# Rodrigops27/MPC-EKF4FastCharge

Measured on AMD Instinct MI355X. Metric: MPC+EKF control steps/sec (whole batch), Np=5 Nc=2; 1/2/4/8 MI355X, higher is better.
Workload: dtype f64

## Files before the change

mpc-ekf4fastcharge_amd/csrc/mpcekf_host.cpp:

```cpp
#include <hip/hip_runtime.h>

#include <sched.h>

#include <algorithm>
#include <cmath>
#include <condition_variable>
#include <cstdarg>
#include <cstdio>
#include <cstdlib>
#include <cstring>
#include <deque>
#include <mutex>
#include <new>
#include <string>
#include <thread>
#include <vector>

#include "../../include/mpcekf.h"
#include "mpcekf_eig.hpp"
#include "mpcekf_kernels.hpp"
#include "mpcekf_summary.hpp"
#include "mpcekf_thermal.hpp"

using namespace mk;
// ... 114 lines not shown
    hipError_t e = err;
    err = hipSuccess;
    return e;
  }
  ~Copier() {
    {
      std::lock_guard<std::mutex> g(mu);
      stop = true;
    }
    cv.notify_all();
    for (std::thread &t : th) t.join();
  }
};

int copy_threads() {
  if (const char *e = std::getenv("MPCEKF_COPY_THREADS")) return std::max(0, std::min(64, std::atoi(e)));
  cpu_set_t set;
  int n = 8;
  if (sched_getaffinity(0, sizeof set, &set) == 0) n = CPU_COUNT(&set);
  return std::max(1, std::min(16, n));
}

}

struct mpcekf_ctx {
  int device = 0;
  hipStream_t stream = nullptr;
  int64_t n = 0;
  int NM = 0, nz = 0, nzp = 0;
  int ncon = 0, ncon_dev = 0, sw = 7;
  bool initialized = false;
  KRom r{};
  KCfg k{};
  KState s{};
  mpcekf_config cfg{};
  double *d_cell_blob = nullptr, *d_plant_blob = nullptr, *d_bulk = nullptr, *d_poly = nullptr;
  double *d_const = nullptr;
  double *d_mb = nullptr;
  bool mb = false;
  double *d_scal = nullptr;
  int *d_int = nullptr;
  double *d_prob = nullptr;
  double *d_zk = nullptr, *d_zbk = nullptr;
  double *d_bnd = nullptr;
  int *d_xm = nullptr;
  double *d_xg = nullptr;
  bool split_cell = false;
  bool quad = false;
  int ekf4_block = 256;
  int *d_ts = nullptr;
  double *d_hist = nullptr;
  double *d_hot = nullptr;
  int *d_hot_i = nullptr;
  int hot_clear() {
    if (d_hot_i) HIPCHK(hipMemsetAsync(d_hot_i, 0xFF, (size_t)n * 4 * sizeof(int), stream));
    return MPCEKF_OK;
  }
  long long *d_stamps = nullptr;
  bool wide = false;
  KWide w{};
  double *d_lin = nullptr, *d_zsoc = nullptr;
  std::vector<double> h_lim;
  double *d_lim = nullptr;
  bool percell = false;
  const double *lim() const { return percell ? d_lim : nullptr; }
  double *d_sum = nullptr, *d_sum_reach = nullptr, *d_sum_obs = nullptr;
  char *d_sum_ring = nullptr;
  int32_t sum_slot = -1;
  size_t sum_row() const { return (((size_t)SUM_WIN * (size_t)n * 8) + 255) & ~(size_t)255; }
  double *d_th = nullptr, *d_th_par = nullptr, *d_th_i = nullptr, *d_th_ocv = nullptr;
  int32_t th_nocv = 0;
  double *d_uk1p = nullptr;
  int flush_period = LAZY_H;
  bool flush_roll = false;
  hipStream_t fstream = nullptr;
  hipEvent_t ev_fork = nullptr, ev_join = nullptr;
  bool bounds_side = false;
  hipEvent_t ev_bfork = nullptr, ev_bjoin = nullptr;
  double *d_tmp = nullptr;
  size_t tmp_bytes = 0;
  char *h_bounce = nullptr;
  size_t h_bytes = 0, bounce_max = (size_t)256 << 20;
  size_t xoff = 0, xchunk = (size_t)4 << 20, xhwm = 0;
  std::vector<hipEvent_t> xev;
  size_t xev_used = 0;
  bool xpending = false;
  Copier *copier = nullptr;
  hipError_t next_event(hipEvent_t *e) {
    if (xev_used == xev.size()) {
      hipEvent_t ne = nullptr;
      hipError_t r = hipEventCreateWithFlags(&ne, hipEventDisableTiming);
      if (r != hipSuccess) return r;
      xev.push_back(ne);
    }
    *e = xev[xev_used++];
    return hipSuccess;
  }
  int drain() {
    hipError_t e = hipStreamSynchronize(stream);
    hipError_t c = copier ? copier->drain() : hipSuccess;
    xoff = 0;
    xev_used = 0;
    xpending = false;
    if (e != hipSuccess) return fail(MPCEKF_E_HIP, "hipStreamSynchronize: %s", hipGetErrorString(e));
    if (c != hipSuccess) return fail(MPCEKF_E_HIP, "output copy: %s", hipGetErrorString(c));
    return MPCEKF_OK;
  }
  bool timing = false;
// ... 657 lines not shown
  hipError_t e = hipStreamCreateWithFlags(&X->stream, hipStreamNonBlocking);
  if (e == hipSuccess && (X->flush_roll || X->bounds_side)) {
    e = hipStreamCreateWithFlags(&X->fstream, hipStreamNonBlocking);
    if (e == hipSuccess) e = hipEventCreateWithFlags(&X->ev_fork, hipEventDisableTiming);
    if (e == hipSuccess) e = hipEventCreateWithFlags(&X->ev_join, hipEventDisableTiming);
    if (e == hipSuccess) e = hipEventCreateWithFlags(&X->ev_bfork, hipEventDisableTiming);
    if (e == hipSuccess) e = hipEventCreateWithFlags(&X->ev_bjoin, hipEventDisableTiming);
  }
  if (e != hipSuccess) { mpcekf_ctx_destroy(X); return fail(MPCEKF_E_HIP, "stream: %s", hipGetErrorString(e)); }
  const size_t n = (size_t)ncells, NM = (size_t)X->NM;
  KState &s = X->s;
  s.n = ncells;
  if ((rc = dalloc(&s.bigx, n * NM * 6)) || (rc = dalloc(&s.ekf, n * NM * REC)) ||
      (rc = dalloc(&X->d_scal, n * 10)) || (rc = dalloc(&s.lam, n * X->ncon_dev)) ||
      (rc = hipMalloc((void **)&X->d_int, (n * 4 + 1) * sizeof(int)) == hipSuccess ? 0 : MPCEKF_E_HIP) || (rc = dalloc(&X->d_prob, n * PROB_DOUBLES)) || (rc = dalloc(&X->d_const, n * 8)) ||
      (rc = dalloc(&X->d_zk, n * (X->nz + 2))) || (rc = dalloc(&X->d_zbk, n * (X->nz + 2))) ||
      (rc = dalloc(&X->d_bnd, n * NBND)) || (rc = dalloc(&X->d_xg, n * 4)) ||
      (rc = hipMalloc((void **)&X->d_xm, n * 4 * sizeof(int)) == hipSuccess ? 0 : MPCEKF_E_HIP) ||
      (rc = dalloc(&X->d_ts, n * NM * 2)) || (rc = dalloc(&X->d_hist, n * LAZY_H * 2)) ||
      (X->mb && (rc = dalloc(&X->d_mb, n * MBREC)))
#ifdef MPCEKF_STAMPS
      || (rc = dalloc(&X->d_stamps, n * NSTAMPS))
#endif
  ) {
    mpcekf_ctx_destroy(X);
    return rc;
  }
  double *sc = X->d_scal;
  s.SOCn = sc; s.SOCp = sc + n; s.x0 = sc + 2 * n; s.S0 = sc + 3 * n; s.priorI = sc + 4 * n;
  s.uk_1 = sc + 5 * n; s.uk = sc + 6 * n; s.vk = sc + 7 * n; s.J_unc = sc + 8 * n; s.J_fin = sc + 9 * n;
  s.warn = X->d_int; s.status = X->d_int + n; s.nviol = X->d_int + 2 * n; s.hflag = X->d_int + 3 * n;
  s.hslow = X->d_int + 4 * n;
  HIPCHK(hipMemset(s.hslow, 0, sizeof(int)));
  s.prob = X->d_prob;
  s.ts_ekf = X->d_ts; s.ts_plant = X->d_ts + n * NM;
  s.hist_p = X->d_hist; s.hist_u = X->d_hist + n * LAZY_H;
  s.mb = X->d_mb;
  s.stamps = X->d_stamps;
  {
    bool hot = true;
    if (const char *e = std::getenv("MPCEKF_HOT_CORNERS")) hot = std::atoi(e) != 0;
    if (hot && !X->mb && !X->quad && !X->flush_roll && n > 0) {
      if (hipMalloc((void **)&X->d_hot, n * 4 * REC * sizeof(double)) != hipSuccess ||
          hipMalloc((void **)&X->d_hot_i, n * 8 * sizeof(int)) != hipSuccess) {
        (void)hipGetLastError();
        if (X->d_hot) (void)hipFree(X->d_hot);
        if (X->d_hot_i) (void)hipFree(X->d_hot_i);
        X->d_hot = nullptr;
        X->d_hot_i = nullptr;
      } else {
        s.hot_rec = X->d_hot;
        s.hot_m = X->d_hot_i;
        s.hot_ts = X->d_hot_i + n * 4;
        if ((rc = X->hot_clear())) { mpcekf_ctx_destroy(X); return rc; }
      }
    }
  }
  if (X->d_stamps) HIPCHK(hipMemset(X->d_stamps, 0, (size_t)n * NSTAMPS * sizeof(long long)));
  double *cs = X->d_const;
  s.Tc = cs; s.SOC0 = cs + n; s.SOC0n = cs + 2 * n; s.SOC0p = cs + 3 * n;
  if (X->sw != 7 && ((rc = dalloc(&X->d_lin, n * MPCEKF_LIN_SIZE)) || (rc = dalloc(&X->d_zsoc, n)))) {
    mpcekf_ctx_destroy(X);
    return rc;
  }
  if (X->wide) {
    KWide &w = X->w;
    w.Np = cfg->Np; w.Nc = cfg->Nc; w.ncon = X->ncon;
    const size_t nc = (size_t)X->ncon;
    if ((rc = dalloc(&w.prob, n * wide_prob_doubles(w.Np, w.Nc))) || (rc = dalloc(&w.X, nc * n * w.Nc)) ||
        (rc = dalloc(&w.R, (size_t)n * (w.Nc * (w.Nc + 1) / 2))) || (rc = dalloc(&w.K, nc * n)) || (rc = dalloc(&w.hii, nc * n)) || (rc = dalloc(&w.it, n)) ||
        (rc = dalloc(&w.smin, (size_t)w.Nc * w.Nc + 1)) || (rc = dalloc(&X->d_lin, n * MPCEKF_LIN_SIZE)) ||
        (rc = dalloc(&w.q, 1)) || (rc = dalloc(&w.list, n)) || (rc = dalloc(&w.hist, 128)) ||
        (rc = dalloc(&X->d_zsoc, n))) {
      mpcekf_ctx_destroy(X);
      return rc;
    }
    HIPCHK(hipMemset(w.q, 0, sizeof(int)));
    HIPCHK(hipMemset(w.hist, 0, 128 * sizeof(int)));
    HIPCHK(hipMemset(w.it, 0, n * sizeof(int)));
    rc = launch_wide_smin(w, -rom->Ts / (3600 * rom->Q), rom->A, X->stream);
    if (rc) { mpcekf_ctx_destroy(X); return fail(MPCEKF_E_HIP, "smin kernel: %s", hipGetErrorString((hipError_t)rc)); }
    HIPCHK(hipStreamSynchronize(X->stream));
  }
  *out = X;
  return MPCEKF_OK;
}

int mpcekf_ctx_destroy(mpcekf_ctx *X) {
  if (!X) return MPCEKF_OK;
  (void)hipSetDevice(X->device);
  if (X->stream) (void)X->drain();
  if (X->fstream) (void)hipStreamSynchronize(X->fstream);
  delete X->copier;
  X->copier = nullptr;
  for (hipEvent_t e : X->xev) (void)hipEventDestroy(e);
  for (hipEvent_t e : X->ev) (void)hipEventDestroy(e);
  if (X->ev_fork) (void)hipEventDestroy(X->ev_fork);
  if (X->ev_join) (void)hipEventDestroy(X->ev_join);
  if (X->ev_bfork) (void)hipEventDestroy(X->ev_bfork);
  if (X->ev_bjoin) (void)hipEventDestroy(X->ev_bjoin);
  void *ptrs[] = {X->d_prob, X->d_cell_blob, X->d_plant_blob, X->d_bulk, X->d_const, X->d_scal, X->d_int, X->d_zk,
                  X->d_zbk,       X->d_tmp,        X->s.bigx, X->s.ekf,   X->s.lam,   X->d_ts, X->d_hist, X->d_stamps, X->d_bnd, X->d_xm, X->d_xg,
                  X->w.prob, X->w.X, X->w.R, X->w.K, X->w.hii, X->w.it, X->w.smin, X->d_lin, X->d_zsoc, X->d_mb, X->d_uk1p,
                  X->w.q, X->w.list, X->w.hist, X->d_poly, X->d_szk, X->d_sxg, X->d_sxm, X->d_slin, X->d_sv, X->d_zslot,
                  X->d_obs_blob, X->d_obs, X->d_obs_plan, X->d_lim, X->d_sum, X->d_sum_reach, X->d_sum_obs,
                  X->d_sum_ring, X->d_th, X->d_th_par, X->d_th_i, X->d_th_ocv, X->d_hot, X->d_hot_i};
  for (void *p : ptrs)
    if (p) (void)hipFree(p);
  for (auto &g : X->graphs) (void)hipGraphExecDestroy(g.exec);
  if (X->h_bounce) (void)hipHostFree(X->h_bounce);
  if (X->fstream) (void)hipStreamDestroy(X->fstream);
  if (X->stream) (void)hipStreamDestroy(X->stream);
  delete X;
  return MPCEKF_OK;
}

int mpcekf_ctx_config(const mpcekf_ctx *X, mpcekf_config *cfg) {
  if (!X || !cfg) return fail(MPCEKF_E_ARG, "ctx_config: null argument");
  *cfg = X->cfg;
  return MPCEKF_OK;
}

int mpcekf_ctx_info(const mpcekf_ctx *X, int64_t *ncells, int32_t *nmodels, int32_t *nz, int32_t *ncon) {
  if (!X) return fail(MPCEKF_E_ARG, "null ctx");
  if (ncells) *ncells = X->n;
  if (nmodels) *nmodels = X->NM;
  if (nz) *nz = X->nz;
  if (ncon) *ncon = X->ncon;
  return MPCEKF_OK;
}

static double host_soc(const mpcekf_ctx *X, int side, double z, double T) {
  const std::vector<double> &tk = X->tabT;
  const int nte = (int)tk.size();
  const std::vector<double> &a = X->soc_end[side][0], &b = X->soc_end[side][1];
  if (nte == 1) return a[0] + z * (b[0] - a[0]);
  const double Tc = std::fmin(std::fmax(T, tk[0]), tk[nte - 1]);
  int j = 0;
  while (j < nte - 2 && Tc >= tk[j + 1]) ++j;
  const double g = (Tc - tk[j]) / (tk[j + 1] - tk[j]);
  const double s0 = a[j] + g * (a[j + 1] - a[j]), s1 = b[j] + g * (b[j + 1] - b[j]);
  return s0 + z * (s1 - s0);
}

static int check_tc(const double *tc, size_t count) {
  for (size_t i = 0; i < count; ++i)
    if (!(tc[i] <= 100) || !std::isfinite(tc[i]))
      return fail(MPCEKF_E_ARG, "temperature %zu = %g: must be finite and in degC (iterEKF.m:62)", i, tc[i]);
  return MPCEKF_OK;
}

static int set_tc(mpcekf_ctx *X, const double *tc, struct Xfer *xf = nullptr);

int mpcekf_init_cells(mpcekf_ctx *X, const double *soc0_pct, const double *tc_degC) {
  if (X) X->stage_zk = X->stage_lin = X->stage_v = X->stage_obs = false;
  if (!X || ((!soc0_pct || !tc_degC) && X->n)) return fail(MPCEKF_E_ARG, "init_cells: null argument");
  HIPCHK(hipSetDevice(X->device));
  const size_t n = (size_t)X->n;
  int rc0 = 0;
// ... 288 lines not shown
      if (slice && fork) HIPCHK(hipStreamWaitEvent(X->stream, X->ev_join, 0));
      if (roll ? t == nsteps : (t % P == 0 || t == nsteps)) {
        const bool timed = E && !roll;
        if (timed) HIPCHK(hipEventRecord(E[5], X->stream));
        if ((rc = lerr(launch_flush(X->r, X->k, X->s, t, t == nsteps ? 0 : t, X->stream), "flush"))) return rc;
        if (timed) HIPCHK(hipEventRecord(E[6], X->stream));
        flushed[k] = timed;
      }
      if (sum && ((size_t)t % ring == 0 || t == nsteps)) {
        KSum q{};
        q.rec = X->d_sum;
        q.reach = X->d_sum_reach;
        q.u = (const double *)f[0].dev;
        q.v = (const double *)f[1].dev;
        q.soc = (const double *)f[2].dev;
        q.phise = (const double *)f[3].dev;
        q.nexec = (const int *)f[4].dev;
        q.obs = (const double *)f[14].dev;
        q.n = X->n;
        q.nrows = (int)((size_t)k % ring) + 1;
        q.max_hild = X->cfg.max_hild;
        if ((rc = lerr(launch_summary(q, X->stream), "summary"))) return rc;
      }
      if (thermal) {
        KTherm q{};
        q.Tc = X->s.Tc;
        q.vk = X->s.vk;
        q.SOCn = X->s.SOCn;
        q.status = X->s.status;
        q.uk = X->s.uk;
        q.iapp = X->d_th_i;
        q.par = X->d_th_par;
        q.ocv = X->d_th_ocv;
        q.rec = X->d_th;
        q.temp = (double *)row(15, k);
        q.heat = (double *)row(16, k);
        q.n = X->n;
        q.nocv = X->th_nocv;
        q.th0n = X->r.th0n;
        q.th100n = X->r.th100n;
        q.Ts = X->r.Ts;
        if ((rc = lerr(launch_thermal(q, X->stream), "thermal"))) return rc;
      }
    }
    return MPCEKF_OK;
  };
  if (capturing) {
    std::vector<uintptr_t> key = {(uintptr_t)nsteps, (uintptr_t)dtc, (uintptr_t)diag, (uintptr_t)bounds};
    for (const F &e : f) key.push_back((uintptr_t)e.dev);
    key.push_back((uintptr_t)osel.plan);
    key.push_back((uintptr_t)nslots);
    key.push_back((uintptr_t)lim);
    key.push_back((uintptr_t)X->s.hot_rec);
    for (int i = 0; i < nslots; ++i) key.push_back((uintptr_t)slots[i]);
    key.push_back((uintptr_t)X->d_th_ocv);
    key.push_back((uintptr_t)X->th_nocv);
    key.push_back((uintptr_t)X->d_th);
    key.push_back((uintptr_t)(sum ? X->d_sum_reach : nullptr));
    key.push_back((uintptr_t)(sum ? X->d_sum : nullptr));
    if ((rc = X->graph_launch(key, run_steps))) return rc;
  } else if ((rc = run_steps())) {
    return rc;
  }
  if (!outputs_on_device)
    for (int i = 0; i < NF; ++i)
      if (f[i].host)
        HIPCHK(hipMemcpyAsync(f[i].host, f[i].dev, per * f[i].width * f[i].esz, hipMemcpyDeviceToHost, X->stream));
  if (nsteps > 0 && f[6].dev)
    HIPCHK(hipMemcpyAsync(X->d_zk, row(6, nsteps - 1), n * nzz * 8, hipMemcpyDeviceToDevice, X->stream));
  if (nsteps > 0 && f[7].dev)
    HIPCHK(hipMemcpyAsync(X->d_zbk, row(7, nsteps - 1), n * nzz * 8, hipMemcpyDeviceToDevice, X->stream));
  HIPCHK(hipStreamSynchronize(X->stream));
  if (X->timing) {
    static const int slot[5] = {MPCEKF_K_PLANT, MPCEKF_K_CELL, MPCEKF_K_BOUNDS, MPCEKF_K_HILD, MPCEKF_K_FLUSH};
    static const int e0[5] = {0, 1, 2, 3, 5};
    for (int k = 0; k < nsteps; ++k)
      for (int j = 0; j < 5; ++j) {
        if ((k + 1) % X->timing_every != 0 && k != nsteps - 1) continue;
        if ((j == 4 && !flushed[k]) || (j == 2 && !bnd_kernel) || (j == 0 && plant_in_cell && !nslots)) continue;
        float ms = 0;
        const int a = j == 3 ? hstart : e0[j], b = j == 3 ? 4 : e0[j] + 1;
        HIPCHK(hipEventElapsedTime(&ms, X->ev[(size_t)k * NEV + a], X->ev[(size_t)k * NEV + b]));
        X->t_ms[slot[j]] += ms;
        X->t_n[slot[j]] += 1;
      }
  }
  return MPCEKF_OK;
}

int mpcekf_step_ex(mpcekf_ctx *X, int32_t nsteps, const double *tc_degC, const mpcekf_traj *tr,
                   int32_t outputs_on_device) {
  return step_impl(X, nsteps, tc_degC, tr, nullptr, 0, nullptr, outputs_on_device);
}

int mpcekf_step_ex_obs(mpcekf_ctx *X, int32_t nsteps, const double *tc_degC, const mpcekf_traj *tr,
                       const int32_t *slots, int32_t nslots, double *obs, int32_t outputs_on_device) {
  return step_impl(X, nsteps, tc_degC, tr, slots, nslots, obs, outputs_on_device);
}

int mpcekf_cl_eig(int32_t n, const double *a, double *re, double *im, double *sv) {
  if (n < 1 || n > mk::eig::MAXN || !a) return fail(MPCEKF_E_ARG, "cl_eig: n must be 1..%d", mk::eig::MAXN);
  double r[mk::eig::MAXN], m[mk::eig::MAXN], s[mk::eig::MAXN];
  if (re || im) mk::eig::eigvals(n, a, r, m);
  if (sv) mk::eig::singvals(n, a, s);
  for (int i = 0; i < n; ++i) {
    if (re) re[i] = r[i];
// ... 1011 lines not shown
```

mpc-ekf4fastcharge_amd/csrc/mpcekf_kernels.hip:

```cpp
#include <hip/hip_runtime.h>

#include <cmath>
#include <cstdlib>
#include <cstdint>
#include <type_traits>

#include "mpcekf_kernels.hpp"
#include "mpcekf_mpc.hpp"
#include "mpcekf_hild.hpp"

#pragma clang fp contract(off)

namespace mk {


#ifdef MPCEKF_STAMPS
#define STAMP(i)                                                                          \
  do {                                                                                    \
    if (io.stamps) io.stamps[(size_t)(i) * s.n + c] = (long long)__builtin_amdgcn_s_memtime(); \
  } while (0)
#define STAMPP(i)                                                                                  \
  do {                                                                                             \
    if (s.stamps) s.stamps[(size_t)(12 + (i)) * s.n + c] = (long long)__builtin_amdgcn_s_memtime(); \
  } while (0)
// ... 941 lines not shown
  }
  if (n2 > 0) {
    double2 v[B];
#pragma unroll
    for (int b = 0; b < B; ++b) v[b] = s2[min(i + b * nt, n2 - 1)];
#pragma unroll
    for (int b = 0; b < B; ++b) d2[min(i + b * nt, n2 - 1)] = v[b];
  }
  if ((len & 1) && threadIdx.x == 0) dst[len - 1] = src[len - 1];
}

#ifndef MPCEKF_RING_CHUNK
#define MPCEKF_RING_CHUNK 8
#endif
constexpr int RCH = MPCEKF_RING_CHUNK;
__device__ __forceinline__ void ring_chunk(const double *ring, const KState &s, int64_t c, int k0, int kmax,
                                           double v[RCH]) {
#pragma unroll
  for (int i = 0; i < RCH; ++i) v[i] = ring[(size_t)(min(k0 + i, kmax) % LAZY_H) * s.n + c];
}
struct PlantCorners {
  int iZu, iZl, iTu, iTl;
};
__device__ __forceinline__ PlantCorners plant_corners(const KRom &r, const double *Tp, const double *Zp,
                                                      double cellSOC, double T) {
  int iZu = 0, iZl = 0, iTu = 0, iTl = 0;
  if (r.nZ > 1) {
    int a, b;
    two_nearest(Zp, r.nZ, cellSOC, a, b);
    iZu = a > b ? a : b; iZl = a < b ? a : b;
  }
  if (r.nT > 1) {
    int a, b;
    two_nearest(Tp, r.nT, T, a, b);
    iTu = a > b ? a : b; iTl = a < b ? a : b;
  }
  return {iZu, iZl, iTu, iTl};
}
__device__ __forceinline__ int corner_model(const KRom &r, const PlantCorners &pc, int j) {
  return ((j & 2) ? pc.iTu : pc.iTl) * r.nZ + ((j & 1) ? pc.iZu : pc.iZl);
}
__device__ __forceinline__ void corner_models(const KRom &r, const PlantCorners &pc, int mm[4]) {
#pragma unroll
  for (int j = 0; j < 4; ++j) mm[j] = corner_model(r, pc, j);
}
__device__ __forceinline__ void plant_weights(const double *Tp, const double *Zp, const PlantCorners &pc,
                                              double cellSOC, double T, double &aZ, double &aT) {
  const double Zu = Zp[pc.iZu], Zl = Zp[pc.iZl], Tu = Tp[pc.iTu], Tl = Tp[pc.iTl];
  aZ = 0.0;
  aT = 0.0;
  if (Zu != Zl) aZ = (cellSOC - Zl) / (Zu - Zl);
  if (Tu != Tl) aT = (T - Tl) / (Tu - Tl);
}
__device__ __forceinline__ void load_corner(const double *bx, double xs[6]) {
  const double2 *p = reinterpret_cast<const double2 *>(bx);
  const double2 q0 = p[0], q1 = p[1], q2 = p[2];
  xs[0] = q0.x; xs[1] = q0.y; xs[2] = q1.x; xs[3] = q1.y; xs[4] = q2.x; xs[5] = q2.y;
}
__device__ __forceinline__ void store_corner(double *bx, const double x[6]) {
  double2 *p = reinterpret_cast<double2 *>(bx);
  p[0] = make_double2(x[0], x[1]);
  p[1] = make_double2(x[2], x[3]);
  p[2] = make_double2(x[4], x[5]);
}
__device__ __forceinline__ void plant_soc_step(const KRom &r, const ETab &et, double SOC0n, double SOC0p, double Iapp,
                                               double &SOCnAvg, double &SOCpAvg) {
  const double Cdleffn = et.f(0, EF_CDL, SOC0n), Cdleffp = et.f(1, EF_CDL, SOC0p);
  double dUn = et.f(0, EF_DU, SOCnAvg), dUp = et.f(1, EF_DU, SOCpAvg);
  double dQn = fabs(r.th100n - r.th0n), dQp = fabs(r.th100p - r.th0p);
  double res0n = -dQn / (3600 * r.Q - Cdleffn * dQn * dUn);
  double res0p = dQp / (3600 * r.Q - Cdleffp * dQp * dUp);
  SOCnAvg = SOCnAvg + res0n * Iapp * r.Ts;
  SOCpAvg = SOCpAvg + res0p * Iapp * r.Ts;
  if (SOCnAvg < 0) SOCnAvg = 0;
  if (SOCnAvg > 1) SOCnAvg = 1;
  if (SOCpAvg < 0) SOCpAvg = 0;
  if (SOCpAvg > 1) SOCpAvg = 1;
}
template <bool A5>
__device__ __forceinline__ void plant_advance(const double *a, const double xs[6], double u, double x[6]) {
#pragma unroll
  for (int e = 0; e < NX; ++e) x[e] = __builtin_fma(a[e], xs[e], u);
  x[NX] = __builtin_fma(A5 ? a[NX] : 1.0, xs[NX], u);
}
template <bool A5>
__device__ __forceinline__ void plant_replay(double xs[6], const double *a, const KState &s, int64_t c, int tsj,
                                             int lazy_t) {
  for (int k0 = tsj + 1; k0 < lazy_t; k0 += RCH) {
    double u[RCH];
    ring_chunk(s.hist_u, s, c, k0, lazy_t - 1, u);
#pragma unroll
    for (int i = 0; i < RCH; ++i)
      if (k0 + i < lazy_t) plant_advance<A5>(a, xs, u[i], xs);
  }
}
__device__ __forceinline__ double plant_row(const double *C, double r0, double d, const double xs[6], double Iapp) {
  double acc = 0.0;
#pragma unroll
  for (int k = 0; k < NX; ++k) acc = acc + C[k] * xs[k];
  acc = acc + r0 * xs[5];
  return acc + d * Iapp;
}
__device__ __forceinline__ double obs_row(const double *B, const double xs[6], double Iapp) {
  const double2 *p = reinterpret_cast<const double2 *>(B);
  const double2 c01 = p[0], c23 = p[1], c4r = p[2], d = p[3];
  double acc = 0.0;
  acc = acc + c01.x * xs[0];
  acc = acc + c01.y * xs[1];
  acc = acc + c23.x * xs[2];
  acc = acc + c23.y * xs[3];
  acc = acc + c4r.x * xs[4];
  acc = acc + c4r.y * xs[5];
  return acc + d.x * Iapp;
}
__device__ __forceinline__ double blend4(double y0, double y1, double y2, double y3, double aZ, double aT) {
  return (1 - aT) * ((1 - aZ) * y0 + aZ * y1) + aT * ((1 - aZ) * y2 + aZ * y3);
// ... 76 lines not shown
  STAMPP(3);
  const double *B = L + mj * PREC;
  double yk[NPLANT];
#pragma unroll
  for (int q = 0; q < NPLANT; ++q) {
    yk[q] = quad_blend(plant_row(B + q * NX, B[NPLANT * NX + q], B[NPLANT * NX + NPLANT + q], xs, Iapp), aZ, aT);
    __builtin_amdgcn_sched_barrier(0);
  }
  STAMPP(4);
  const double V = plant_vcell(r, et, yk, T, Iapp, negSOC, posSOC, SOC0n, SOC0p);
  STAMPP(5);
  if (j == 0) {
    s.SOCn[c] = SOCnAvg;
    s.SOCp[c] = SOCpAvg;
    vout[c] = V;
  }
  if (lazy_t && tsj < lazy_t) {
    double x[6];
    plant_advance<true>(a, xs, Iapp, x);
    store_corner(bx, x);
    s.ts_plant[c * r.NM + mj] = lazy_t;
  }
  STAMPP(6);
}

struct ObsBlob {
  const double *tb, *L, *Tp, *Zp;
};
template <bool GR>
__device__ __forceinline__ ObsBlob obs_stage(const KObs &o, double *lds) {
  const int lo = GR ? o.tab : 0;
  stage_lds(lds, o.blob + lo, o.len - lo);
  __syncthreads();
  const double *tb = lds - lo;
  const double *Tp = tb + o.tab + o.tablen;
  return {tb, GR ? o.blob : lds, Tp, Tp + MAXT};
}
struct ObsCell {
  double negSOC, posSOC, SOC0n, SOC0p, cellSOC, aZ, aT;
  ETab et;
  double xs[6];
  const double *B;
  int mj;
};
template <bool PL>
__device__ __forceinline__ void obs_cell(const KRom &r, const KState &s, const KObs &o, const ObsBlob &ob, int64_t c,
                                         int j, double T, ObsCell &k, int *tsj = nullptr) {
  k.negSOC = s.SOCn[c], k.posSOC = s.SOCp[c];
  k.SOC0n = s.SOC0n[c], k.SOC0p = s.SOC0p[c];
  k.et = etab<PL>(r, ob.tb + o.tab, T);
  k.cellSOC = (k.negSOC - r.th0n) / (r.th100n - r.th0n);
  const PlantCorners pc = plant_corners(r, ob.Tp, ob.Zp, k.cellSOC, T);
  k.mj = corner_model(r, pc, j);
  load_corner(s.bigx + ((size_t)c * r.NM + k.mj) * 6, k.xs);
  if (tsj) *tsj = s.ts_plant[c * r.NM + k.mj];
  plant_weights(ob.Tp, ob.Zp, pc, k.cellSOC, T, k.aZ, k.aT);
  k.B = ob.L + (size_t)k.mj * o.stride;
}
__device__ __forceinline__ double obs_correct(int kind, double v, const ObsCell &k, double UocpnAvg, double UocppAvg,
                                              double negPhise0, double V) {
  switch (kind) {
    case OBS_NTHSS: return fmin(fmax(v + k.SOC0n, 1e-6), 1 - 1e-6);
    case OBS_PTHSS: return fmin(fmax(v + k.SOC0p, 1e-6), 1 - 1e-6);
    case OBS_NPHISE: return v + UocpnAvg;
    case OBS_PPHISE: return v + UocppAvg;
    case OBS_PHIE: return v - negPhise0;
    case OBS_THETAE: return fmax(v + 1, 1e-6);
    case OBS_PPHIS: return v + V;
    default: return v;
  }
}
constexpr int OBS_BLOCK = 512;
template <bool GR, bool PL>
__global__ void __launch_bounds__(OBS_BLOCK) k_plant_obs(const KRom r, const KState s, const KObs o,
                                                            const double *iapp) {
  extern __shared__ double lds[];
  const int64_t gt = (int64_t)blockIdx.x * blockDim.x + threadIdx.x;
  const int j = (int)(gt & 3);
  const int64_t c = gt >> 2;
  const ObsBlob ob = obs_stage<GR>(o, lds);
  if (c >= s.n) return;
  const size_t n = (size_t)s.n;
  double *rec = o.rec + c;
  auto put = [&](int slot, double v) {
    if ((slot & 3) == j) rec[(size_t)slot * n] = v;
  };
  if (s.status[c] & ST_ERROR) {
    for (int k = j; k < o.nobs; k += 4) rec[(size_t)k * n] = __builtin_nan("");
    return;
  }
  const double Iapp = iapp[c];
  const double T = s.Tc[c] + 273.15;
  ObsCell k;
  obs_cell<PL>(r, s, o, ob, c, j, T, k);
  double yk[R_PHISE0 + 1];
#pragma unroll
  for (int q = 0; q <= R_PHISE0; ++q) {
    yk[q] = quad_blend(obs_row(k.B + q * OBS_ROW, k.xs, Iapp), k.aZ, k.aT);
    __builtin_amdgcn_sched_barrier(0);
  }
  const double V = plant_vcell(r, k.et, yk, T, Iapp, k.negSOC, k.posSOC, k.SOC0n, k.SOC0p);
  __builtin_amdgcn_sched_barrier(0);
  const double UocpnAvg = k.et.f(0, EF_U, k.negSOC), UocppAvg = k.et.f(1, EF_U, k.posSOC);
  const double negPhise0 = yk[R_PHISE0] + UocpnAvg;
  __builtin_amdgcn_sched_barrier(0);
  put(OBS_S_NEGSOC, k.negSOC);
  put(OBS_S_POSSOC, k.posSOC);
  put(OBS_S_CELLSOC, k.cellSOC);
// ... 85 lines not shown
  for (int64_t c = blockIdx.x; c < s.n; c += gridDim.x) {
    if (do_ekf) {
      double pri = s.priorI[c];
      double2 *base = reinterpret_cast<double2 *>(s.ekf + (size_t)c * ne);
      for (int j = threadIdx.x; j < ne / 2; j += blockDim.x) {
        int e0 = (2 * j) % REC;
        double2 v = base[j];
        double add0 = e0 < NX ? pri : W;
        double add1 = e0 + 1 < NX ? pri : W;
        v.x = __builtin_fma(cC[2 * j], v.x, add0);
        v.y = __builtin_fma(cC[2 * j + 1], v.y, add1);
        base[j] = v;
      }
    }
    if (do_plant) {
      double u = iapp[c];
      double2 *base = reinterpret_cast<double2 *>(s.bigx + (size_t)c * np);
      for (int j = threadIdx.x; j < np / 2; j += blockDim.x) {
        double2 v = base[j];
        v.x = __builtin_fma(cP[2 * j], v.x, u);
        v.y = __builtin_fma(cP[2 * j + 1], v.y, u);
        base[j] = v;
      }
    }
  }
}

__device__ __forceinline__ double rl64(double v, int l) {
  const long long b = __double_as_longlong(v);
  const int lo = __builtin_amdgcn_readlane((int)b, l), hi = __builtin_amdgcn_readlane((int)(b >> 32), l);
  return __longlong_as_double(((long long)hi << 32) | (long long)(unsigned)lo);
}
__global__ void __launch_bounds__(256) k_flush(const KRom r, const KCfg cf, const KState s, const int t,
                                               const int new_ts, const int64_t c_lo, const int64_t c_hi) {
  const int NM = r.NM;
  const int lane = threadIdx.x & 63;
  const int64_t nw = (int64_t)gridDim.x * (blockDim.x >> 6);
  const int64_t w0 = ((int64_t)blockIdx.x * blockDim.x + threadIdx.x) >> 6;
  const double W = cf.SigmaW;
  const double *cC = r.bulk_tab, *cP = r.bulk_tab + (size_t)NM * REC;
  for (int m0 = 0; m0 < NM; m0 += 64) {
    const int m = m0 + lane;
    const bool act = m < NM;
    const int mm = act ? m : NM - 1;
    double ce[REC], cp[6];
#pragma unroll
    for (int e = 0; e < REC; ++e) ce[e] = cC[(size_t)mm * REC + e];
#pragma unroll
    for (int e = 0; e < 6; ++e) cp[e] = cP[(size_t)mm * 6 + e];
    struct FCell {
      double hpl, hul, xe[REC], xp[6];
      int tse, tsp;
      int slot;
    };
    auto fload = [&](int64_t c, FCell &F) {
      F.hpl = s.hist_p[(size_t)(lane & (LAZY_H - 1)) * s.n + c];
      F.hul = s.hist_u[(size_t)(lane & (LAZY_H - 1)) * s.n + c];
      F.slot = -1;
      if (s.hot_m) {
#pragma unroll
        for (int j = 0; j < 4; ++j)
          if (act && s.hot_m[(size_t)j * s.n + c] == m) F.slot = j;
      }
      const int *tp = F.slot >= 0 ? s.hot_ts + (size_t)F.slot * s.n + c : s.ts_ekf + c * NM + mm;
      F.tse = (act && !(cf.flags & KF_MB)) ? *tp : t;
      F.tsp = act ? s.ts_plant[c * NM + m] : t;
      const double2 *re = reinterpret_cast<const double2 *>(F.slot >= 0 ? hot_slot(s, F.slot, c)
                                                                        : s.ekf + ((size_t)c * NM + mm) * REC);
      const size_t rst = F.slot >= 0 ? (size_t)s.n : 1;
      const double2 *rp = reinterpret_cast<const double2 *>(s.bigx + ((size_t)c * NM + mm) * 6);
#pragma unroll
      for (int e = 0; e < REC / 2; ++e) {
        const double2 v = re[e * rst];
        F.xe[2 * e] = v.x;
        F.xe[2 * e + 1] = v.y;
      }
#pragma unroll
      for (int e = 0; e < 3; ++e) {
        const double2 v = rp[e];
        F.xp[2 * e] = v.x;
        F.xp[2 * e + 1] = v.y;
      }
    };
    FCell cur;
    if (c_lo + w0 < c_hi) fload(c_lo + w0, cur);
    for (int64_t c = c_lo + w0; c < c_hi; c += nw) {
      FCell nx;
      if (c + nw < c_hi) fload(c + nw, nx);
      const double hpl = cur.hpl, hul = cur.hul;
      const int tse = cur.tse, tsp = cur.tsp;
      double2 *re = reinterpret_cast<double2 *>(s.ekf + ((size_t)c * NM + mm) * REC);
      double2 *rp = reinterpret_cast<double2 *>(s.bigx + ((size_t)c * NM + mm) * 6);
      double *xe = cur.xe, *xp = cur.xp;
      int kmin = min(tse, tsp);
#pragma unroll
      for (int o = 1; o < 64; o <<= 1) kmin = min(kmin, __shfl_xor(kmin, o));
      for (int k = kmin + 1; k <= t; ++k) {
        const int sl = k & (LAZY_H - 1);
        const double p = rl64(hpl, sl), u = rl64(hul, sl);
        if (k > tse) {
#pragma unroll
          for (int e = 0; e < NX; ++e) xe[e] = __builtin_fma(ce[e], xe[e], p);
#pragma unroll
          for (int e = NX; e < REC; ++e) xe[e] = __builtin_fma(ce[e], xe[e], W);
        }
        if (k > tsp) {
#pragma unroll
          for (int e = 0; e < 6; ++e) xp[e] = __builtin_fma(cp[e], xp[e], u);
        }
      }
      if (tse < t || cur.slot >= 0) {
#pragma unroll
        for (int e = 0; e < REC / 2; ++e) re[e] = make_double2(xe[2 * e], xe[2 * e + 1]);
      }
      if (cur.slot >= 0) s.hot_m[(size_t)cur.slot * s.n + c] = -1;
      if (tsp < t) {
#pragma unroll
        for (int e = 0; e < 3; ++e) rp[e] = make_double2(xp[2 * e], xp[2 * e + 1]);
      }
      if (act) {
        s.ts_ekf[c * NM + m] = new_ts;
        s.ts_plant[c * NM + m] = new_ts;
      }
      cur = nx;
    }
  }
}

__device__ __forceinline__ void replay_x(double x[NX], const double *a, int ts, int t, double pt, const KState &s,
                                        int64_t c) {
  if (ts + 1 < t) {
    for (int k0 = ts + 1; k0 < t; k0 += RCH) {
      double p[RCH];
      ring_chunk(s.hist_p, s, c, k0, t - 1, p);
#pragma unroll
      for (int i = 0; i < RCH; ++i)
        if (k0 + i < t)
#pragma unroll
          for (int e = 0; e < NX; ++e) x[e] = __builtin_fma(a[e], x[e], p[i]);
    }
  }
  if (ts < t)
#pragma unroll
    for (int e = 0; e < NX; ++e) x[e] = __builtin_fma(a[e], x[e], pt);
}
__device__ __forceinline__ void replay_S(double S[NPK], const double *a, int ts, int t, double W) {
  for (int k = ts + 1; k <= t; ++k) {
#pragma unroll
    for (int i = 0, pp = 0; pp < NX; ++pp)
#pragma unroll
      for (int q = pp; q < NX; ++q, ++i) S[i] = __builtin_fma(a[NX + i], S[i], W);
  }
}

template <int NZ>
__device__ __forceinline__ void ekf_catch_up4(const KState &s, const CellCtx &cc, int NM, const int m[4], int64_t c,
                                              int t, double W, double pt, const bool held[4]) {
  int ts[4];
#pragma unroll
  for (int j = 0; j < 4; ++j) ts[j] = held[j] ? t : s.ts_ekf[c * NM + m[j]];
  bool need[4];
#pragma unroll
  for (int j = 0; j < 4; ++j) {
    need[j] = ts[j] < t;
#pragma unroll
    for (int i = 0; i < j; ++i) need[j] = need[j] && m[i] != m[j];
  }
  if (!(need[0] || need[1] || need[2] || need[3])) return;
  double x[4][NX], S[4][NPK];
// ... 163 lines not shown
    return;
  }
  double V[NA6 * NA6], w[NA6];
  jacobi6(a, V);
#pragma unroll
  for (int k = 0; k < NA6; ++k) w[k] = fabs(a[pk6(k, k)]);
#pragma unroll
  for (int rr = 0; rr < NA6; ++rr)
#pragma unroll
    for (int cI = rr; cI < NA6; ++cI) {
      double hrc = 0.0, hcr = 0.0;
#pragma unroll
      for (int k = 0; k < NA6; ++k) {
        hrc = hrc + (V[rr * NA6 + k] * w[k]) * V[cI * NA6 + k];
        hcr = hcr + (V[cI * NA6 + k] * w[k]) * V[rr * NA6 + k];
      }
      double v = (((P[rr * NA6 + cI] + P[cI * NA6 + rr]) + hrc) + hcr) / 4.0;
      if (bump) v = v * 2.0;
      S[rr * NA6 + cI] = v;
      S[cI * NA6 + rr] = v;
    }
}

__device__ __forceinline__ double qform(const double T[NPK], const double rw[NX]) {
  double q = 0.0;
#pragma unroll
  for (int k = 0; k < NX; ++k) {
    double u = T[pk(k, k)] * rw[k];
#pragma unroll
    for (int l = k + 1; l < NX; ++l) u = __builtin_fma(T[pk(k, l)], rw[l], u);
    q = k == 0 ? rw[0] * u : __builtin_fma(rw[k], u, q);
  }
  return q;
}

template <int NZ, bool PL>
__device__ __forceinline__ double cell_plant(const KRom &r, const KState &s, const double *L, const double *tb,
                                             const double *Tp, const double *Zp, int64_t c, int lazy_t, double Iapp,
                                             double tcs, int st, double &ring_p) {
  constexpr int OA = NZ * NX + NZ, OR0 = NZ * NX + NZ + NX + NPK, OD = NZ * NX;
  const int stride = r.cell_stride;
  if (lazy_t) ring_p = s.priorI[c];
  if (st & ST_ERROR) return __builtin_nan("");
  const double T = tcs + 273.15;
  const ETab et = etab<PL>(r, tb + r.cell_tab, T);
  double SOCnAvg = s.SOCn[c], SOCpAvg = s.SOCp[c];
  const double SOC0n = s.SOC0n[c], SOC0p = s.SOC0p[c];
  const double negSOC = SOCnAvg, posSOC = SOCpAvg;
  double cellSOC = (SOCnAvg - r.th0n) / (r.th100n - r.th0n);
  const PlantCorners pc = plant_corners(r, Tp, Zp, cellSOC, T);
  int mm[4];
  corner_models(r, pc, mm);
  double *bx = s.bigx + (size_t)c * r.NM * 6;
  double xs[4][6];
  int tsj[4] = {0, 0, 0, 0};
#pragma unroll
  for (int j = 0; j < 4; ++j) {
    load_corner(bx + (size_t)mm[j] * 6, xs[j]);
    if (lazy_t) tsj[j] = s.ts_plant[c * r.NM + mm[j]];
  }
  plant_soc_step(r, et, SOC0n, SOC0p, Iapp, SOCnAvg, SOCpAvg);
  if (lazy_t) {
#pragma unroll
    for (int j = 0; j < 4; ++j) plant_replay<false>(xs[j], L + mm[j] * stride + OA, s, c, tsj[j], lazy_t);
  }
  double y[4][NPLANT];
#pragma unroll
  for (int j = 0; j < 4; ++j) {
    const double *B = L + mm[j] * stride;
#pragma unroll
    for (int q = 0; q < NPLANT; ++q) {
      y[j][q] = plant_row(B + q * NX, B[OR0 + q], B[OD + q], xs[j], Iapp);
      launder(y[j][q]);
    }
    __builtin_amdgcn_sched_barrier(0);
  }
  double aZ, aT;
  plant_weights(Tp, Zp, pc, cellSOC, T, aZ, aT);
  double yk[NPLANT];
#pragma unroll
  for (int q = 0; q < NPLANT; ++q) yk[q] = blend4(y[0][q], y[1][q], y[2][q], y[3][q], aZ, aT);
  const double V = plant_vcell(r, et, yk, T, Iapp, negSOC, posSOC, SOC0n, SOC0p);
  s.SOCn[c] = SOCnAvg;
  s.SOCp[c] = SOCpAvg;
  if (lazy_t) {
#pragma unroll
    for (int j = 0; j < 4; ++j) {
      if (tsj[j] >= lazy_t) continue;
      double x[6];
      plant_advance<false>(L + mm[j] * stride + OA, xs[j], Iapp, x);
      store_corner(bx + (size_t)mm[j] * 6, x);
      s.ts_plant[c * r.NM + mm[j]] = lazy_t;
    }
  }
  return V;
}

template <int NZ, int PARTS, bool MB = false, bool GR = false, bool PL = false>
__global__ void __launch_bounds__(256) k_cell(const KRom r, const KCfg cf, const KState s, const KIO io) {
  extern __shared__ double lds[];
  const int lo = GR ? r.cell_tab : 0;
  stage_lds(lds, r.cell_blob + lo, r.cell_len - lo);
  __syncthreads();
  const double *tb = lds - lo;
  const double *Tp = tb + r.cell_tab + r.cell_tablen;
  const double *Zp = Tp + MAXT;
  const int64_t c = (int64_t)blockIdx.x * blockDim.x + threadIdx.x;
  double ring_u = 0.0, ring_p = 0.0;
  bool ring_late = false;
  auto body = [&]() {
  if (c >= s.n) return;
  const int nz = r.nz;
  const double NaN = __builtin_nan("");
  CellCtx cc;
  cc.L = GR ? r.cell_blob : lds;
  cc.Tp = Tp;
  cc.Zp = Zp;
  cc.erec = s.ekf + (size_t)c * r.NM * REC;
  cc.stride = r.cell_stride;
  const bool fplant = (PARTS & P_EKF) && !MB && io.plant;
  const double Tc = fplant && io.tc_in ? io.tc_in[c] : s.Tc[c];
  if (fplant && io.tc_in) s.Tc[c] = Tc;
  cc.T = Tc > 100 ? Tc : Tc + 273.15;
  cc.et = etab<PL>(r, tb + r.cell_tab, cc.T);
  int st = s.status[c];
  const bool fused = io.mode & MODE_FUSED;
  if (io.mode & (MODE_MPC | MODE_FUSED)) s.hflag[c] = 0;
  STAMP(0);

  auto fail_outputs = [&]() {
    if (io.u) io.u[c] = NaN;
    if (io.v) io.v[c] = NaN;
    if (io.soc) io.soc[c] = NaN;
    if (io.phise) io.phise[c] = NaN;
    if (io.nexec) io.nexec[c] = 0;
    if (io.zk)
      for (int q = 0; q < nz + 2; ++q) io.zk[c * (nz + 2) + q] = NaN;
    if (io.zbk)
      for (int q = 0; q < nz + 2; ++q) io.zbk[c * (nz + 2) + q] = NaN;
    if (io.bnd) io.bnd[BD_M * s.n + c] = -1.0;
    if (io.uk_out) io.uk_out[c] = NaN;
    if (io.x_out)
      for (int q = 0; q < 6; ++q) io.x_out[c * 6 + q] = NaN;
    if (io.junc_out) io.junc_out[c] = NaN;
    if (io.jfin_out) io.jfin_out[c] = NaN;
// ... 1529 lines not shown
```

mpc-ekf4fastcharge_amd/csrc/mpcekf_kernels.hpp:

```cpp
#pragma once
#include <cstddef>
#include <cstdint>

namespace mk {

constexpr int NX = 5;
constexpr int NPK = 15;
constexpr int NA = 7;
constexpr int REC = 20;
constexpr int MAXT = 8;
constexpr int MAXZ = 40;
constexpr int MAXROWS = 64;
constexpr int NPLANT = 9;
constexpr int PREC = NPLANT * NX + NPLANT + NPLANT + 6;
#ifndef MPCEKF_LAZY_H
#define MPCEKF_LAZY_H 64
#endif
constexpr int LAZY_H = MPCEKF_LAZY_H;
constexpr int MAXTT = 8;
constexpr int MBREC = 42;
constexpr int KF_MB = 1 << 8;

enum { R_IFDL0 = 0, R_IFDL3, R_IF0, R_IF3, R_TH0, R_TH3, R_TE1, R_TEE, R_PHIE, R_PHISE0, R_NPHISE2, NROLE };
enum : unsigned { G_NTH = 1, G_PTH = 2, G_NPHISE = 4, G_PPHISE = 8, G_PHIE = 16, G_PHIE0 = 32, G_THETAE = 64,
// ... 1 lines not shown
enum { C0_ZERO = 0, C0_CHATV0, C0_RES0N, C0_RES0P, C0_DUN, C0_DUP, C0_MDUN };
enum { ST_ERROR = 1, ST_LOCKOUT = 2, ST_THETAE_NEG = 4 };

struct KRom {
  int NM, nT, nZ, nz, nzp;
  int nth, nte;
  double Ts, Q, F, R, Rc, Tref;
  double th0n, th100n, th0p, th100p;
  unsigned char flags[MAXROWS];
  unsigned fmask[8];
  unsigned char c0k[MAXROWS];
  short perm[MAXROWS];
  const double *cell_blob;
  int cell_stride, cell_tab, cell_tablen, cell_len;
  const double *plant_blob;
  int plant_tab, plant_tablen, plant_len;
  const double *bulk_tab;
  int rom_global;
  int cell_plant;
  int npoly, arr, nodes;
  const double *poly;
};
constexpr int KPOLY = 6;
constexpr int KDESC = 4;
constexpr int KMAP = 4;

struct KCfg {
  double SigmaV, SigmaW, ref, u_max, u_min, du_min, du_max, v_max, phise_min, zmax, hild_tol;
  int max_warn, max_hild, flags;
};

enum { LK_REF = 0, LK_U_MAX, LK_U_MIN, LK_DU_MIN, LK_DU_MAX, LK_V_MAX, LK_PHISE_MIN, LK_ZMAX, NLIMK };

struct KState {
  int64_t n;
  double *bigx;
  double *ekf;
  double *SOCn, *SOCp, *x0, *S0, *priorI, *uk_1, *uk, *vk;
  double *lam;
  int *warn, *status;
  double *Tc;
  const double *SOC0, *SOC0n, *SOC0p;
  double *J_unc, *J_fin;
  int *nviol;
  int *hflag;
  int *hslow;
  double *prob;
  double *mb;
  int *ts_ekf, *ts_plant;
  double *hist_p, *hist_u;
  long long *stamps;
  double *hot_rec;
  int *hot_m, *hot_ts;
};
constexpr int HOT_PAIRS = REC / 2;

constexpr int OBS_ROW = 8;
constexpr int OBS_MAXROWS = 32;
enum { OBS_PLAIN = 0, OBS_NTHSS, OBS_PTHSS, OBS_NPHISE, OBS_PPHISE, OBS_PHIE, OBS_THETAE, OBS_PPHIS };
enum { OBS_S_NEGSOC = 0, OBS_S_POSSOC, OBS_S_CELLSOC };
struct KObs {
  const double *blob;
  int stride, tab, tablen, len;
  int global;
  int nobs, slot_phie0;
  unsigned desc[OBS_MAXROWS];
  double *rec;
};

enum { OBS_SRC_NEGSOC = -1, OBS_SRC_POSSOC = -2, OBS_SRC_CELLSOC = -3, OBS_SRC_PHIE0 = -4, OBS_SRC_VCELL = -5 };
enum { OBS_NEED_V = 1,
       OBS_NEED_UN = 2,
       OBS_NEED_UP = 4 };
struct KObsSel {
  const int *plan;
  int nsel, need;
  double *out;
};

struct KIO {
  int mode;
  double *u, *v, *soc, *phise;
  int *nexec;
  double *zk, *zbk;
  const double *vk_in, *ik_in;
  int *xm_out; double *xg_out;
  const double *zk_in; const int *xm_in; const double *xg_in;
  double *lin_out; const double *lin_in;
  const double *soc_k1_in; double *uk_out;
  int lazy_t;
  double *bnd;
  long long *stamps;
  double *zsoc_out;
  double *x_out;
  double *junc_out, *jfin_out, *normdu_out;
  int *nviol_out;
  int plant;
  const double *tc_in;
};
constexpr int NSTAMPS = 20;
enum { BD_G = 0, BD_M = 4, BD_K = 8, BD_C0 = 14, BD_R0N, BD_R0P, BD_DUN, BD_DUP, BD_S0, NBND };

enum { MODE_EKF = 1, MODE_LIN = 2, MODE_MPC = 4, MODE_FUSED = 8 };
enum { P_EKF = 1, P_MPC = 2, P_ALL = 3, P_LIN = 4 };

struct KWide {
  int Np, Nc, ncon;
  double *prob;
// ... 68 lines not shown
```

Baseline: 269.2 million.

## Add hot-corner cache for plant state in SoA layout

Adds a per-cell four-slot cache for the plant model's active corner states, stored structure-of-arrays (strided by n) so accesses coalesce across cells, mirroring the existing EKF hot-corner cache. On a tag hit the plant step reads and writes the cached slots, and on a miss it spills them back to the bigx array. The flush kernel now checks both EKF and plant tags through lane broadcasts and prefetches the next cell's tags. This adds tag checks, spill logic and extra memory, and risks divergence when cells frequently change corners.

```diff
diff --git a/mpc-ekf4fastcharge_amd/csrc/mpcekf_host.cpp b/mpc-ekf4fastcharge_amd/csrc/mpcekf_host.cpp
--- a/mpc-ekf4fastcharge_amd/csrc/mpcekf_host.cpp
+++ b/mpc-ekf4fastcharge_amd/csrc/mpcekf_host.cpp
@@ -190,8 +190,11 @@
   double *d_hist = nullptr;
   double *d_hot = nullptr;
   int *d_hot_i = nullptr;
+  double *d_hotp = nullptr;
+  int *d_hotp_i = nullptr;
   int hot_clear() {
     if (d_hot_i) HIPCHK(hipMemsetAsync(d_hot_i, 0xFF, (size_t)n * 4 * sizeof(int), stream));
+    if (d_hotp_i) HIPCHK(hipMemsetAsync(d_hotp_i, 0xFF, (size_t)n * 4 * sizeof(int), stream));
     return MPCEKF_OK;
   }
   long long *d_stamps = nullptr;
@@ -955,9 +958,25 @@
         s.hot_rec = X->d_hot;
         s.hot_m = X->d_hot_i;
         s.hot_ts = X->d_hot_i + n * 4;
-        if ((rc = X->hot_clear())) { mpcekf_ctx_destroy(X); return rc; }
       }
     }
+    bool hotp = true;
+    if (const char *e = std::getenv("MPCEKF_HOT_PLANT")) hotp = std::atoi(e) != 0;
+    if (hotp && !X->mb && !X->quad && !X->flush_roll && X->r.cell_plant && n > 0) {
+      if (hipMalloc((void **)&X->d_hotp, n * 4 * 6 * sizeof(double)) != hipSuccess ||
+          hipMalloc((void **)&X->d_hotp_i, n * 8 * sizeof(int)) != hipSuccess) {
+        (void)hipGetLastError();
+        if (X->d_hotp) (void)hipFree(X->d_hotp);
+        if (X->d_hotp_i) (void)hipFree(X->d_hotp_i);
+        X->d_hotp = nullptr;
+        X->d_hotp_i = nullptr;
+      } else {
+        s.hotp_x = X->d_hotp;
+        s.hotp_m = X->d_hotp_i;
+        s.hotp_ts = X->d_hotp_i + n * 4;
+      }
+    }
+    if ((rc = X->hot_clear())) { mpcekf_ctx_destroy(X); return rc; }
   }
   if (X->d_stamps) HIPCHK(hipMemset(X->d_stamps, 0, (size_t)n * NSTAMPS * sizeof(long long)));
   double *cs = X->d_const;
@@ -1007,7 +1026,7 @@
                   X->w.prob, X->w.X, X->w.R, X->w.K, X->w.hii, X->w.it, X->w.smin, X->d_lin, X->d_zsoc, X->d_mb, X->d_uk1p,
                   X->w.q, X->w.list, X->w.hist, X->d_poly, X->d_szk, X->d_sxg, X->d_sxm, X->d_slin, X->d_sv, X->d_zslot,
                   X->d_obs_blob, X->d_obs, X->d_obs_plan, X->d_lim, X->d_sum, X->d_sum_reach, X->d_sum_obs,
-                  X->d_sum_ring, X->d_th, X->d_th_par, X->d_th_i, X->d_th_ocv, X->d_hot, X->d_hot_i};
+                  X->d_sum_ring, X->d_th, X->d_th_par, X->d_th_i, X->d_th_ocv, X->d_hot, X->d_hot_i, X->d_hotp, X->d_hotp_i};
   for (void *p : ptrs)
     if (p) (void)hipFree(p);
   for (auto &g : X->graphs) (void)hipGraphExecDestroy(g.exec);
@@ -1402,6 +1421,7 @@
     key.push_back((uintptr_t)nslots);
     key.push_back((uintptr_t)lim);
     key.push_back((uintptr_t)X->s.hot_rec);
+    key.push_back((uintptr_t)X->s.hotp_x);
     for (int i = 0; i < nslots; ++i) key.push_back((uintptr_t)slots[i]);
     key.push_back((uintptr_t)X->d_th_ocv);
     key.push_back((uintptr_t)X->th_nocv);
diff --git a/mpc-ekf4fastcharge_amd/csrc/mpcekf_kernels.hip b/mpc-ekf4fastcharge_amd/csrc/mpcekf_kernels.hip
--- a/mpc-ekf4fastcharge_amd/csrc/mpcekf_kernels.hip
+++ b/mpc-ekf4fastcharge_amd/csrc/mpcekf_kernels.hip
@@ -1017,16 +1017,26 @@
   if (Zu != Zl) aZ = (cellSOC - Zl) / (Zu - Zl);
   if (Tu != Tl) aT = (T - Tl) / (Tu - Tl);
 }
-__device__ __forceinline__ void load_corner(const double *bx, double xs[6]) {
+__device__ __forceinline__ void load_corner(const double *bx, double xs[6], size_t st = 1) {
   const double2 *p = reinterpret_cast<const double2 *>(bx);
-  const double2 q0 = p[0], q1 = p[1], q2 = p[2];
+  const double2 q0 = p[0], q1 = p[st], q2 = p[2 * st];
   xs[0] = q0.x; xs[1] = q0.y; xs[2] = q1.x; xs[3] = q1.y; xs[4] = q2.x; xs[5] = q2.y;
 }
-__device__ __forceinline__ void store_corner(double *bx, const double x[6]) {
+__device__ __forceinline__ void store_corner(double *bx, const double x[6], size_t st = 1) {
   double2 *p = reinterpret_cast<double2 *>(bx);
   p[0] = make_double2(x[0], x[1]);
-  p[1] = make_double2(x[2], x[3]);
-  p[2] = make_double2(x[4], x[5]);
+  p[st] = make_double2(x[2], x[3]);
+  p[2 * st] = make_double2(x[4], x[5]);
+}
+__device__ __forceinline__ double *hotp_slot(const KState &s, int j, int64_t c) {
+  return s.hotp_x + 2 * ((size_t)j * HOTP_PAIRS * (size_t)s.n + (size_t)c);
+}
+__device__ __forceinline__ int hotp_find(const KState &s, int64_t c, int m) {
+  int slot = -1;
+#pragma unroll
+  for (int i = 0; i < 4; ++i)
+    if (s.hotp_m[(size_t)i * s.n + c] == m) slot = i;
+  return slot;
 }
 __device__ __forceinline__ void plant_soc_step(const KRom &r, const ETab &et, double SOC0n, double SOC0p, double Iapp,
                                                double &SOCnAvg, double &SOCpAvg) {
@@ -1209,8 +1219,10 @@
   k.cellSOC = (k.negSOC - r.th0n) / (r.th100n - r.th0n);
   const PlantCorners pc = plant_corners(r, ob.Tp, ob.Zp, k.cellSOC, T);
   k.mj = corner_model(r, pc, j);
-  load_corner(s.bigx + ((size_t)c * r.NM + k.mj) * 6, k.xs);
-  if (tsj) *tsj = s.ts_plant[c * r.NM + k.mj];
+  const int slot = tsj && s.hotp_m ? hotp_find(s, c, k.mj) : -1;
+  load_corner(slot >= 0 ? hotp_slot(s, slot, c) : s.bigx + ((size_t)c * r.NM + k.mj) * 6, k.xs,
+              slot >= 0 ? (size_t)s.n : 1);
+  if (tsj) *tsj = *(slot >= 0 ? s.hotp_ts + (size_t)slot * s.n + c : s.ts_plant + c * r.NM + k.mj);
   plant_weights(ob.Tp, ob.Zp, pc, k.cellSOC, T, k.aZ, k.aT);
   k.B = ob.L + (size_t)k.mj * o.stride;
 }
@@ -1402,41 +1414,55 @@
       double hpl, hul, xe[REC], xp[6];
       int tse, tsp;
       int slot;
+      int pslot;
     };
-    auto fload = [&](int64_t c, FCell &F) {
+    const int *tags = lane < 4 ? s.hot_m : s.hotp_m;
+    auto ftag = [&](int64_t c) -> int { return lane < 8 && tags ? tags[(size_t)(lane & 3) * s.n + c] : -1; };
+    auto fload = [&](int64_t c, FCell &F, const int tag) {
       F.hpl = s.hist_p[(size_t)(lane & (LAZY_H - 1)) * s.n + c];
       F.hul = s.hist_u[(size_t)(lane & (LAZY_H - 1)) * s.n + c];
       F.slot = -1;
-      if (s.hot_m) {
-#pragma unroll
-        for (int j = 0; j < 4; ++j)
-          if (act && s.hot_m[(size_t)j * s.n + c] == m) F.slot = j;
+      F.pslot = -1;
+#pragma unroll
+      for (int j = 0; j < 4; ++j) {
+        if (act && __builtin_amdgcn_readlane(tag, j) == m) F.slot = j;
+        if (act && __builtin_amdgcn_readlane(tag, 4 + j) == m) F.pslot = j;
       }
       const int *tp = F.slot >= 0 ? s.hot_ts + (size_t)F.slot * s.n + c : s.ts_ekf + c * NM + mm;
+      const int *tq = F.pslot >= 0 ? s.hotp_ts + (size_t)F.pslot * s.n + c : s.ts_plant + c * NM + mm;
       F.tse = (act && !(cf.flags & KF_MB)) ? *tp : t;
-      F.tsp = act ? s.ts_plant[c * NM + m] : t;
+      F.tsp = act ? *tq : t;
       const double2 *re = reinterpret_cast<const double2 *>(F.slot >= 0 ? hot_slot(s, F.slot, c)
                                                                         : s.ekf + ((size_t)c * NM + mm) * REC);
-      const size_t rst = F.slot >= 0 ? (size_t)s.n : 1;
-      const double2 *rp = reinterpret_cast<const double2 *>(s.bigx + ((size_t)c * NM + mm) * 6);
-#pragma unroll
-      for (int e = 0; e < REC / 2; ++e) {
-        const double2 v = re[e * rst];
+      const double2 *rp = reinterpret_cast<const double2 *>(F.pslot >= 0 ? hotp_slot(s, F.pslot, c)
+                                                                         : s.bigx + ((size_t)c * NM + mm) * 6);
+      const size_t rst = F.slot >= 0 ? (size_t)s.n : 1, pst = F.pslot >= 0 ? (size_t)s.n : 1;
+#pragma unroll
+      for (int e = 0; e < REC / 2; ++e, re += rst) {
+        const double2 v = *re;
         F.xe[2 * e] = v.x;
         F.xe[2 * e + 1] = v.y;
       }
 #pragma unroll
-      for (int e = 0; e < 3; ++e) {
-        const double2 v = rp[e];
+      for (int e = 0; e < 3; ++e, rp += pst) {
+        const double2 v = *rp;
         F.xp[2 * e] = v.x;
         F.xp[2 * e + 1] = v.y;
       }
     };
     FCell cur;
-    if (c_lo + w0 < c_hi) fload(c_lo + w0, cur);
+    int tagn = -1;
+    if (c_lo + w0 < c_hi) {
+      fload(c_lo + w0, cur, ftag(c_lo + w0));
+      if (c_lo + w0 + nw < c_hi) tagn = ftag(c_lo + w0 + nw);
+    }
     for (int64_t c = c_lo + w0; c < c_hi; c += nw) {
       FCell nx;
-      if (c + nw < c_hi) fload(c + nw, nx);
+      if (c + nw < c_hi) {
+        const int tag = tagn;
+        if (c + 2 * nw < c_hi) tagn = ftag(c + 2 * nw);
+        fload(c + nw, nx, tag);
+      }
       const double hpl = cur.hpl, hul = cur.hul;
       const int tse = cur.tse, tsp = cur.tsp;
       double2 *re = reinterpret_cast<double2 *>(s.ekf + ((size_t)c * NM + mm) * REC);
@@ -1464,7 +1490,8 @@
         for (int e = 0; e < REC / 2; ++e) re[e] = make_double2(xe[2 * e], xe[2 * e + 1]);
       }
       if (cur.slot >= 0) s.hot_m[(size_t)cur.slot * s.n + c] = -1;
-      if (tsp < t) {
+      if (cur.pslot >= 0) s.hotp_m[(size_t)cur.pslot * s.n + c] = -1;
+      if (tsp < t || cur.pslot >= 0) {
 #pragma unroll
         for (int e = 0; e < 3; ++e) rp[e] = make_double2(xp[2 * e], xp[2 * e + 1]);
       }
@@ -1734,12 +1761,35 @@
   int mm[4];
   corner_models(r, pc, mm);
   double *bx = s.bigx + (size_t)c * r.NM * 6;
+  const size_t hn = (size_t)s.n;
+  bool hot = false, hit = false;
+  if (s.hotp_m != nullptr && lazy_t != 0) {
+    int hm[4];
+#pragma unroll
+    for (int j = 0; j < 4; ++j) hm[j] = s.hotp_m[j * hn + c];
+    hot = pc.iZu != pc.iZl && pc.iTu != pc.iTl;
+    hit = hot && hm[0] == mm[0] && hm[1] == mm[1] && hm[2] == mm[2] && hm[3] == mm[3];
+    if (!hit) {
+#pragma unroll 1
+      for (int j = 0; j < 4; ++j) {
+        const int mh = s.hotp_m[j * hn + c];
+        if (mh < 0) continue;
+        double xh[6];
+        load_corner(hotp_slot(s, j, c), xh, hn);
+        store_corner(bx + (size_t)mh * 6, xh);
+        s.ts_plant[c * r.NM + mh] = s.hotp_ts[j * hn + c];
+        if (!hot) s.hotp_m[j * hn + c] = -1;
+      }
+    }
+  }
+  const size_t rst = hit ? hn : 1;
+  const size_t wst = hot ? hn : 1;
   double xs[4][6];
   int tsj[4] = {0, 0, 0, 0};
 #pragma unroll
   for (int j = 0; j < 4; ++j) {
-    load_corner(bx + (size_t)mm[j] * 6, xs[j]);
-    if (lazy_t) tsj[j] = s.ts_plant[c * r.NM + mm[j]];
+    load_corner(hit ? hotp_slot(s, j, c) : bx + (size_t)mm[j] * 6, xs[j], rst);
+    if (lazy_t) tsj[j] = *(hit ? s.hotp_ts + j * hn + c : s.ts_plant + c * r.NM + mm[j]);
   }
   plant_soc_step(r, et, SOC0n, SOC0p, Iapp, SOCnAvg, SOCpAvg);
   if (lazy_t) {
@@ -1768,11 +1818,15 @@
   if (lazy_t) {
 #pragma unroll
     for (int j = 0; j < 4; ++j) {
-      if (tsj[j] >= lazy_t) continue;
+      if (tsj[j] >= lazy_t) {
+        if (hot && !hit) s.hotp_m[j * hn + c] = -1;
+        continue;
+      }
       double x[6];
       plant_advance<false>(L + mm[j] * stride + OA, xs[j], Iapp, x);
-      store_corner(bx + (size_t)mm[j] * 6, x);
-      s.ts_plant[c * r.NM + mm[j]] = lazy_t;
+      store_corner(hot ? hotp_slot(s, j, c) : bx + (size_t)mm[j] * 6, x, wst);
+      *(hot ? s.hotp_ts + j * hn + c : s.ts_plant + c * r.NM + mm[j]) = lazy_t;
+      if (hot && !hit) s.hotp_m[j * hn + c] = mm[j];
     }
   }
   return V;
diff --git a/mpc-ekf4fastcharge_amd/csrc/mpcekf_kernels.hpp b/mpc-ekf4fastcharge_amd/csrc/mpcekf_kernels.hpp
--- a/mpc-ekf4fastcharge_amd/csrc/mpcekf_kernels.hpp
+++ b/mpc-ekf4fastcharge_amd/csrc/mpcekf_kernels.hpp
@@ -77,8 +77,11 @@
   long long *stamps;
   double *hot_rec;
   int *hot_m, *hot_ts;
+  double *hotp_x;
+  int *hotp_m, *hotp_ts;
 };
 constexpr int HOT_PAIRS = REC / 2;
+constexpr int HOTP_PAIRS = 3;
 
 constexpr int OBS_ROW = 8;
 constexpr int OBS_MAXROWS = 32;
```

New measurement: 274.1 million, median of 6. +1.8%, better.
